# jesselasse/MARL-DMFB

Measured on AMD Instinct MI355X. Metric: env-steps/sec (whole node), 10x10 DMFB 4-droplet fov9, higher is better.
Workload: dtype int8 env state/obs + f64 rewards; fp32 Q-net; 1 GPU; DMFB 10x10, drop_num=4, fov=9, 4096 parallel envs per GPU (BASELINE configs[1]); parallelism=dp1: chips sharded per rank, one flat RCCL all-reduce per learn

## Files before the change

__graft_entry__.py:

```python
import os
import subprocess
import sys

ROOT = os.path.dirname(os.path.abspath(__file__))
if ROOT not in sys.path:
    sys.path.insert(0, ROOT)


def build():
    jobs = str(max(1, min(8, os.cpu_count() or 1)))
    env = dict(os.environ, PYTORCH_ROCM_ARCH='gfx950')
    subprocess.check_call(['make', '-C', os.path.join(ROOT, 'marl_dmfb_amd', 'csrc'), '-j', jobs, '-s'], env=env)
    subprocess.check_call(['make', '-C', os.path.join(ROOT, 'oracle'), '-s'], env=env)
    import marl_dmfb_amd
    from marl_dmfb_amd import _lib
    lib = _lib.dmfb_vec()
    for name in _lib.DMFB_VEC_SYMBOLS:
        getattr(lib, name)
    lib = _lib.meda_vec()
    for name in _lib.MEDA_VEC_SYMBOLS:
        getattr(lib, name)
    lib = _lib.crnn_ops()
    for name in ('crnn_conv9_forward', 'crnn_front9_forward', 'crnn_front19_forward', 'crnn_front_padded_cols', 'crnn_conv9_backward', 'crnn_conv19_backward', 'crnn_front9_forward_live', 'gru_seq_forward', 'gru_seq_backward', 'gru_seq_forward_packed', 'gru_seq_backward_packed'):
        getattr(lib, name)
    lib = _lib.crnn_fov()
    for name in _lib.SIGNATURES['crnn_fov']:
        getattr(lib, name)
    lib = _lib.crnn_wide()
    for name in _lib.SIGNATURES['crnn_wide']:
        getattr(lib, name)
    lib = _lib.rollout_ops()
    for name in ('rollout_select_actions', 'rollout_post_step', 'rollout_gru_head_select_stream', 'rollout_stream_step'):
        getattr(lib, name)
    lib = _lib.vdn_ops()
    for name in ('vdn_td_forward', 'vdn_td_backward', 'vdn_td_forward_packed', 'vdn_td_backward_packed', 'vdn_gather_units', 'vdn_clip_adam_step'):
        getattr(lib, name)
    for name in list(_lib.SIGNATURES['vdn_tail']) + list(_lib.SIGNATURES['vdn_lambda']) + list(_lib.SIGNATURES['vdn_double']):
        getattr(lib, name)
    lib = _lib.qmix_ops()
    for name in list(_lib.SIGNATURES['qmix_ops']) + list(_lib.SIGNATURES['qmix_packed']) + list(_lib.SIGNATURES['qmix_lambda']) + \
            list(_lib.SIGNATURES['qmix_double']):
        getattr(lib, name)
    lib = _lib.route_plan()
    for name in _lib.SIGNATURES['route_plan']:
        getattr(lib, name)
    lib = _lib.meda_plan()
# ... 82 lines not shown
```

marl_dmfb_amd/_lib.py:

```python
import ctypes as C
import os

_HERE = os.path.dirname(os.path.abspath(__file__))
LIB_DIR = os.path.join(_HERE, 'lib')
_CACHE = {}
_FILE = {'rollout_route': 'rollout_ops', 'vdn_tail': 'vdn_ops', 'vdn_lambda': 'vdn_ops', 'vdn_double': 'vdn_ops',
         'qmix_packed': 'qmix_ops', 'qmix_lambda': 'qmix_ops', 'qmix_double': 'qmix_ops'}


class HipLibraryMissing(RuntimeError):
    pass


def load(name):
    if name in _CACHE:
        return _CACHE[name]
    stem = _FILE.get(name, name)
    path = os.path.join(LIB_DIR, 'lib%s%s.so' % (stem, os.environ.get('MARL_DMFB_VARIANT_' + stem.upper(), '')))
    if not os.path.exists(path):
        raise HipLibraryMissing(
            '%s not found: build the HIP extension first (python -c "import __graft_entry__ as g; g.build()" '
            'or make -C marl_dmfb_amd/csrc). There is no CPU fallback.' % path)
    import torch
    lib = C.CDLL(path)
    _CACHE[name] = lib
    return lib


class DmfbVecConfig(C.Structure):
# ... 128 lines not shown
        'crnn_wide_last_hip_error': ([], i32),
    },
    'crnn_ops': {
        'crnn_conv9_forward': [vp, i64, i64, vp, vp, vp, vp, i32, vp, i64, vp],
        'crnn_front9_forward': [vp, i64, vp, i32, i64, vp, vp, vp, vp, vp, vp, i32, vp, i64, i32, vp],
        'crnn_front9_forward_live': [vp, i64, vp, i32, i64, vp, vp, vp, vp, vp, vp, i32, vp, i64, i32, vp, vp, i32, vp],
        'crnn_front19_forward': [vp, i64, vp, i32, i64, vp, vp, vp, vp, vp, vp, i32, vp, i64, i32, vp],
        'crnn_front_padded_cols': ([i32], i32),
        'crnn_conv9_backward_parts': ([i32], i32),
        'crnn_conv9_backward': [vp, i64, i64, vp, i64, vp, i64, vp, vp, vp, i32, vp, i32, vp, vp],
        'crnn_mlp_backward_parts': ([], i32),
        'crnn_mlp_backward': [vp, i64, i32, vp, i32, i64, vp, i64, vp, i64, i32, vp, vp, vp, vp],
        'crnn_conv19_backward_parts': ([i32], i32),
        'crnn_conv19_backward': [vp, i64, i64, vp, i64, vp, i64, vp, vp, vp, vp, i32, vp, i32, vp, vp],
        'crnn_last_hip_error': ([], i32),
        'gru_seq_forward': [vp, vp, vp, vp, vp, i32, i64, i32, vp, vp, vp],
        'gru_seq_backward': [vp, vp, vp, vp, vp, i32, i64, i32, vp, vp, vp, vp, vp],
        'gru_seq_forward_packed': [vp, vp, vp, vp, vp, i32, i64, i32, _i32p, vp, vp, vp],
        'gru_seq_forward_packed_pair': [vp] * 14 + [i32, i64, i32, _i32p, vp],
        'gru_seq_backward_packed': [vp, vp, vp, vp, vp, i32, i64, i32, _i32p, vp, vp, vp, vp, vp, vp],
        'gru_seq_row_blocks': ([i64], i64),
        'gru_last_hip_error': ([], i32),
    },
    'rollout_ops': {
        'rollout_select_actions': [vp, i32, i32, i32, vp, i32, u64, vp, vp, vp, vp, vp, i32, i32, vp],
        'rollout_gru_head_select': [vp, vp, vp, vp, vp, vp, vp, i32, i32, i32, i32, vp, i32, u64, vp, vp, vp, vp, vp, i32, i32, vp, vp],
        'rollout_gru_head_select_live': [vp, vp, vp, vp, vp, vp, vp, i32, i32, i32, i32, vp, i32, u64, vp, vp, vp, vp, vp, i32, i32, vp, vp,
                                         vp, vp],
        'rollout_compact_alive': [i32, vp, vp, vp, vp],
        'rollout_post_step': [i32, i32, i32, vp, vp, vp, vp, i32, vp, vp, vp, vp, vp, vp, vp, vp, vp, f32, f32, vp, vp, vp, i32, vp, vp,
                              vp],
        'rollout_gru_head_select_stream': [vp, vp, vp, vp, vp, vp, vp, i32, i32, i32, i32, vp, i32, u64, vp, vp, vp, vp, vp, i32, vp, vp,
                                           vp],
        'rollout_stream_step': [i32, i32, i32, i32, i32, i32, vp, vp, vp, vp, vp, vp, i32, vp, C.POINTER(RolloutStage),
                                C.POINTER(RolloutRing), i32, vp, vp, vp, f32, f32, vp, vp],
        'rollout_last_hip_error': ([], i32),
    },
    'rollout_route': {
        'rollout_route_select': [i32, i32, i32, i32, vp, vp, vp, i32, vp, vp, vp, vp, vp, vp],
        'rollout_last_hip_error': ([], i32),
    },
    'route_plan': {
        'route_plan_dmfb': [i32, i32, i32, i32, i32, vp, vp, vp, vp, vp, vp, vp, vp, vp, vp, vp],
        'route_follow_dmfb': [i32] * 6 + [vp] * 16,
        'route_plan_dmfb_opt': [i32] * 5 + [vp] * 10 + [i32, i32, vp],
        'route_follow_dmfb_opt': [i32] * 6 + [vp] * 15 + [i32, i32, vp],
# ... 193 lines not shown
    return _CACHE[key]


def dmfb_vec():
    return _library('dmfb_vec')


def meda_vec():
    return _library('meda_vec')


def crnn_ops():
    return _library('crnn_ops')


def crnn_fov():
    return _library('crnn_fov')


def crnn_wide():
    return _library('crnn_wide')


def rollout_ops():
    return _library('rollout_ops')


def rollout_route():
    return _library('rollout_route')


def route_plan():
    return _library('route_plan')


def meda_plan():
    return _library('meda_plan')


def meda_follow():
    return _library('meda_follow')


def meda_plan_wide():
    return _library('meda_plan_wide')

# ... 36 lines not shown
```

marl_dmfb_amd/csrc/gru_ops.hip:

```cpp
#include <hip/hip_runtime.h>

#include <cstdint>
#include <cstdio>
#include <cstdlib>

#include "../../include/crnn_ops.h"

#define HIP_ABI_TAG "crnn_ops"
#define HIP_ABI_ERR CRNN_ERR_HIP
#include "hip_abi.h"

namespace {

constexpr int kBlock = 512;
constexpr int H = 128;
constexpr int RW = 8;
constexpr int KQ = 32;

__device__ __forceinline__ float sigmoidf_(float x) { return 1.0f / (1.0f + __expf(-x)); }

struct SeqOff {
    int32_t packed;
    int32_t off[GRU_SEQ_MAX_STEPS + 1];
};

typedef float f32x2 __attribute__((ext_vector_type(2)));
typedef float f32x4 __attribute__((ext_vector_type(4)));

__global__ __launch_bounds__(kBlock) void k_gru_seq_fwd(const float *__restrict__ igates, const float *__restrict__ h0,
// ... 57 lines not shown
            const int rr = ra + s;
            if (rr < rvt) {
                const float hr = s_part[0][rr][0][u] + s_part[1][rr][0][u] + s_part[2][rr][0][u] + s_part[3][rr][0][u];
                const float hz = s_part[0][rr][1][u] + s_part[1][rr][1][u] + s_part[2][rr][1][u] + s_part[3][rr][1][u];
                const float hn = s_part[0][rr][2][u] + s_part[1][rr][2][u] + s_part[2][rr][2][u] + s_part[3][rr][2][u] + bhn;
                const float rg = sigmoidf_(ig[s][0] + hr + bir);
                const float zg = sigmoidf_(ig[s][1] + hz + biz);
                const float ng = tanhf(ig[s][2] + bin + rg * hn);
                const float hp = s_h[rr >> 1][u][rr & 1];
                const float hnew = (1.0f - zg) * ng + zg * hp;
                const size_t o = base + row0 + rr;
                hs[o * H + u] = hnew;
                if (gates) {
                    gates[o * 4 * H + u] = rg; gates[o * 4 * H + H + u] = zg; gates[o * 4 * H + 2 * H + u] = ng;
                    gates[o * 4 * H + 3 * H + u] = hn;
                }
                s_h[rr >> 1][u][rr & 1] = hnew;
            }
        }
        __syncthreads();
    }
}

__global__ __launch_bounds__(kBlock) void k_gru_seq_bwd(const float *__restrict__ grad_hs, const float *__restrict__ gates,
                                                        const float *__restrict__ hs, const float *__restrict__ h0,
                                                        const float *__restrict__ w_hh, int T, long R,
                                                        float *__restrict__ d_ig, float *__restrict__ d_hg,
                                                        float *__restrict__ d_h0, float *__restrict__ bias_part, const SeqOff so,
                                                        float *__restrict__ h_prev_out) {
    __shared__ __attribute__((aligned(16))) float s_dhg[RW / 2][3][H][2];
    __shared__ __attribute__((aligned(16))) float s_part[4][RW][H];
    const int tid = threadIdx.x, q = tid / H, u = tid - q * H;
    const long row0 = (long)blockIdx.x * RW;
    const int rv = (int)min((long)RW, R - row0);
    f32x4 wt[3][KQ / 4];
#pragma unroll
    for (int g = 0; g < 3; ++g)
#pragma unroll
        for (int k = 0; k < KQ / 4; ++k) {
            const float *col = w_hh + (size_t)(g * H + q * KQ + 4 * k) * H + u;
            wt[g][k] = (f32x4){col[0], col[H], col[2 * H], col[3 * H]};
        }
    const int ra = 2 * q;
    float gh[2] = {0.0f, 0.0f};
    float bs_r = 0.0f, bs_z = 0.0f, bs_n = 0.0f, bs_hn = 0.0f;
    int t_last = -1;
    for (int t = 0; t < T; ++t)
        if (row0 < (so.packed ? (long)(so.off[t + 1] - so.off[t]) : R)) t_last = t;
    struct In { float g, rg, zg, ng, hn, hp; };
    In cur[2], nx[2];
    auto fetch = [&](int t, In (&in)[2]) __attribute__((always_inline)) {
        const long rt = so.packed ? (long)(so.off[t + 1] - so.off[t]) : R;
        const int rvt = (int)min((long)rv, rt - row0);
        const size_t base = so.packed ? (size_t)so.off[t] : (size_t)t * R;
        const size_t base_prev = so.packed ? (size_t)so.off[t > 0 ? t - 1 : 0] : (size_t)(t > 0 ? t - 1 : 0) * R;
#pragma unroll
        for (int s = 0; s < 2; ++s) {
            const int rr = ra + s;
            const bool on = rr < rvt;
            const size_t o = base + row0 + (on ? rr : 0);
            in[s].g = on ? grad_hs[o * H + u] : 0.0f;
            in[s].rg = on ? gates[o * 4 * H + u] : 0.0f;
            in[s].zg = on ? gates[o * 4 * H + H + u] : 0.0f;
            in[s].ng = on ? gates[o * 4 * H + 2 * H + u] : 0.0f;
            in[s].hn = on ? gates[o * 4 * H + 3 * H + u] : 0.0f;
            in[s].hp = !on ? 0.0f : t > 0 ? hs[(base_prev + row0 + rr) * H + u] : h0 ? h0[(row0 + rr) * H + u] : 0.0f;
        }
    };
    if (t_last >= 0) fetch(t_last, cur);
    for (int t = t_last; t >= 0; --t) {
        const long rt = so.packed ? (long)(so.off[t + 1] - so.off[t]) : R;
        const int rvt = (int)min((long)rv, rt - row0);
        const size_t base = so.packed ? (size_t)so.off[t] : (size_t)t * R;
        float direct[2];
#pragma unroll
        for (int s = 0; s < 2; ++s) {
            const int rr = ra + s;
            float dpr = 0.0f, dpz = 0.0f, dpn = 0.0f, dhn = 0.0f;
            direct[s] = 0.0f;
            if (rr < rvt) {
                const size_t o = base + row0 + rr;
                const float g = cur[s].g + gh[s];
                const float rg = cur[s].rg, zg = cur[s].zg, ng = cur[s].ng, hn = cur[s].hn;
                const float hp = cur[s].hp;
                if (h_prev_out) h_prev_out[o * H + u] = hp;
                const float dn = g * (1.0f - zg), dz = g * (hp - ng);
                direct[s] = g * zg;
                dpn = dn * (1.0f - ng * ng);
                dhn = dpn * rg;
                dpr = dpn * hn * rg * (1.0f - rg);
                dpz = dz * zg * (1.0f - zg);
                d_ig[o * 3 * H + u] = dpr; d_ig[o * 3 * H + H + u] = dpz; d_ig[o * 3 * H + 2 * H + u] = dpn;
// ... 3 lines not shown
            s_dhg[rr >> 1][0][u][rr & 1] = dpr; s_dhg[rr >> 1][1][u][rr & 1] = dpz; s_dhg[rr >> 1][2][u][rr & 1] = dhn;
        }
        if (t > 0) fetch(t - 1, nx);
        __syncthreads();
#pragma unroll
        for (int rp = 0; rp < RW / 2; ++rp) {
            f32x2 acc = {0.0f, 0.0f};
#pragma unroll
            for (int g = 0; g < 3; ++g) {
                const f32x4 *pd = (const f32x4 *)(&s_dhg[rp][g][q * KQ][0]);
#pragma unroll
                for (int j = 0; j < KQ / 4; ++j) {
                    const f32x4 v0 = pd[2 * j], v1 = pd[2 * j + 1], wv = wt[g][j];
                    acc = __builtin_elementwise_fma((f32x2){wv.x, wv.x}, (f32x2){v0.x, v0.y}, acc);
                    acc = __builtin_elementwise_fma((f32x2){wv.y, wv.y}, (f32x2){v0.z, v0.w}, acc);
                    acc = __builtin_elementwise_fma((f32x2){wv.z, wv.z}, (f32x2){v1.x, v1.y}, acc);
                    acc = __builtin_elementwise_fma((f32x2){wv.w, wv.w}, (f32x2){v1.z, v1.w}, acc);
                }
            }
            s_part[q][2 * rp][u] = acc.x;
            s_part[q][2 * rp + 1][u] = acc.y;
        }
        __syncthreads();
#pragma unroll
        for (int s = 0; s < 2; ++s) {
            const int rr = ra + s;
            gh[s] = direct[s] + s_part[0][rr][u] + s_part[1][rr][u] + s_part[2][rr][u] + s_part[3][rr][u];
            cur[s] = nx[s];
        }
    }
    if (d_h0)
#pragma unroll
        for (int s = 0; s < 2; ++s)
            if (ra + s < rv) d_h0[(row0 + ra + s) * H + u] = gh[s];
    if (bias_part) {
        __syncthreads();
        s_part[q][0][u] = bs_r; s_part[q][1][u] = bs_z; s_part[q][2][u] = bs_n; s_part[q][3][u] = bs_hn;
        __syncthreads();
        if (q == 0) {
            float v[4];
#pragma unroll
            for (int k = 0; k < 4; ++k) v[k] = (s_part[0][k][u] + s_part[1][k][u]) + (s_part[2][k][u] + s_part[3][k][u]);
            float *bp = bias_part + (size_t)blockIdx.x * 6 * H;
            bp[u] = v[0]; bp[H + u] = v[1]; bp[2 * H + u] = v[2];
            bp[3 * H + u] = v[0]; bp[4 * H + u] = v[1]; bp[5 * H + u] = v[3];
        }
    }
}

constexpr int kMW = 16, kMHS = 132;
struct GruNetIO {
    const float *igates, *h0, *w_hh, *b_ih, *b_hh;
    float *hs, *gates;
};
__global__ __launch_bounds__(kBlock) void k_gru_seq_fwd_mfma(GruNetIO n0, GruNetIO n1, int blocks_per_net, int T, long R, const SeqOff so) {
    __shared__ __attribute__((aligned(16))) float s_h[2][kMW][kMHS];
    const bool second = (int)blockIdx.x >= blocks_per_net;
    const GruNetIO io = second ? n1 : n0;
    const long row0 = (long)((int)blockIdx.x - (second ? blocks_per_net : 0)) * kMW;
    const int tid = threadIdx.x, lane = tid & 63, wave = tid >> 6, j = lane & 15, kq = lane >> 4;
    const int u = 16 * wave + j;
    const int rv = (int)min((long)kMW, R - row0);
    f32x4 bw[3][8];
#pragma unroll
    for (int g = 0; g < 3; ++g)
#pragma unroll
        for (int jj = 0; jj < 8; ++jj) bw[g][jj] = *(const f32x4 *)(io.w_hh + (size_t)(g * H + u) * H + 16 * jj + 4 * kq);
    const float bir = io.b_ih[u] + io.b_hh[u], biz = io.b_ih[H + u] + io.b_hh[H + u], bin = io.b_ih[2 * H + u], bhn = io.b_hh[2 * H + u];
    for (int i = tid; i < kMW * H; i += kBlock) {
        const int rr = i / H, c = i - rr * H;
        s_h[0][rr][c] = (rr < rv && io.h0) ? io.h0[(row0 + rr) * H + c] : 0.0f;
        s_h[1][rr][c] = 0.0f;
    }
    __syncthreads();
    for (int t = 0; t < T; ++t) {
        const long rt = so.packed ? (long)(so.off[t + 1] - so.off[t]) : R;
        if (row0 >= rt) break;
        const int rvt = (int)min((long)rv, rt - row0);
        const size_t base = (so.packed ? (size_t)so.off[t] : (size_t)t * R) + (size_t)row0;
        const float (*cur)[kMHS] = s_h[t & 1];
        float (*nxt)[kMHS] = s_h[(t + 1) & 1];
        float ig[4][3];
#pragma unroll
        for (int q = 0; q < 4; ++q) {
            const int rr = 4 * kq + q;
#pragma unroll
            for (int g = 0; g < 3; ++g) ig[q][g] = rr < rvt ? io.igates[(base + rr) * 3 * H + g * H + u] : 0.0f;
        }
        f32x4 a4[8];
#pragma unroll
        for (int jj = 0; jj < 8; ++jj) a4[jj] = *(const f32x4 *)(&cur[j][16 * jj + 4 * kq]);
        f32x4 acc2[2][3];
#pragma unroll
        for (int hlf = 0; hlf < 2; ++hlf)
#pragma unroll
            for (int g = 0; g < 3; ++g) acc2[hlf][g] = f32x4{0.0f, 0.0f, 0.0f, 0.0f};
#pragma unroll
        for (int jj = 0; jj < 4; ++jj)
#pragma unroll
            for (int c = 0; c < 4; ++c)
#pragma unroll
                for (int hlf = 0; hlf < 2; ++hlf)
#pragma unroll
                    for (int g = 0; g < 3; ++g)
                        acc2[hlf][g] = __builtin_amdgcn_mfma_f32_16x16x4f32(a4[4 * hlf + jj][c], bw[g][4 * hlf + jj][c], acc2[hlf][g], 0, 0, 0);
        f32x4 acc[3];
#pragma unroll
        for (int g = 0; g < 3; ++g) acc[g] = acc2[0][g] + acc2[1][g];
#pragma unroll
        for (int q = 0; q < 4; ++q) {
            const int rr = 4 * kq + q;
            if (rr < rvt) {
                const float hn = acc[2][q] + bhn;
                const float rg = sigmoidf_(ig[q][0] + acc[0][q] + bir);
                const float zg = sigmoidf_(ig[q][1] + acc[1][q] + biz);
                const float ng = tanhf(ig[q][2] + bin + rg * hn);
                const float hp = cur[rr][u];
                const float hnew = (1.0f - zg) * ng + zg * hp;
                const size_t o = base + rr;
                io.hs[o * H + u] = hnew;
                if (io.gates) {
                    io.gates[o * 4 * H + u] = rg; io.gates[o * 4 * H + H + u] = zg; io.gates[o * 4 * H + 2 * H + u] = ng;
                    io.gates[o * 4 * H + 3 * H + u] = hn;
                }
                nxt[rr][u] = hnew;
            }
        }
        __syncthreads();
    }
}

}

extern "C" {

static int make_seq_off(const int32_t *step_rows, int T, int64_t R, SeqOff &so) {
    so.packed = step_rows ? 1 : 0;
    if (!step_rows) return CRNN_OK;
    if (T > GRU_SEQ_MAX_STEPS) return CRNN_ERR_UNSUPPORTED;
    long off = 0, prev = R;
    for (int t = 0; t < T; ++t) {
        if (step_rows[t] < 0 || step_rows[t] > prev) return CRNN_ERR_BAD_ARG;
        so.off[t] = (int32_t)off;
        off += step_rows[t];
        prev = step_rows[t];
        if (off > 0x7fffffffL) return CRNN_ERR_BAD_ARG;
    }
    so.off[T] = (int32_t)off;
    return CRNN_OK;
}

// ... 18 lines not shown
int gru_seq_forward_packed(const float *d_igates, const float *d_h0, const float *d_w_hh, const float *d_b_ih, const float *d_b_hh,
                           int T, int64_t R, int hidden, const int32_t *step_rows, float *d_hs, float *d_gates, void *stream) {
    if (!step_rows) return CRNN_ERR_BAD_ARG;
    return seq_forward(d_igates, d_h0, d_w_hh, d_b_ih, d_b_hh, T, R, hidden, step_rows, d_hs, d_gates, stream);
}

int gru_seq_forward_packed_pair(const float *d_igates_a, const float *d_h0_a, const float *d_w_hh_a, const float *d_b_ih_a,
                                const float *d_b_hh_a, float *d_hs_a, float *d_gates_a, const float *d_igates_b, const float *d_h0_b,
                                const float *d_w_hh_b, const float *d_b_ih_b, const float *d_b_hh_b, float *d_hs_b, float *d_gates_b,
                                int T, int64_t R, int hidden, const int32_t *step_rows, void *stream) {
    if (!d_igates_a || !d_w_hh_a || !d_b_ih_a || !d_b_hh_a || !d_hs_a || T < 0 || R < 0 || !step_rows) return CRNN_ERR_BAD_ARG;
    const bool two = d_igates_b != nullptr;
    if (two && (!d_w_hh_b || !d_b_ih_b || !d_b_hh_b || !d_hs_b)) return CRNN_ERR_BAD_ARG;
    if ((((size_t)d_w_hh_a | (size_t)d_w_hh_b) & 15) != 0) return CRNN_ERR_BAD_ARG;
    if (hidden != H) return CRNN_ERR_UNSUPPORTED;
    if (T == 0 || R == 0) return CRNN_OK;
    SeqOff so;
    const int rc = make_seq_off(step_rows, T, R, so);
    if (rc != CRNN_OK) return rc;
    const long per_net = (R + kMW - 1) / kMW;
    if (per_net * 2 > 0x7fffffffL) return CRNN_ERR_BAD_ARG;
    const GruNetIO a{d_igates_a, d_h0_a, d_w_hh_a, d_b_ih_a, d_b_hh_a, d_hs_a, d_gates_a};
    const GruNetIO b{d_igates_b, d_h0_b, d_w_hh_b, d_b_ih_b, d_b_hh_b, d_hs_b, d_gates_b};
    LAUNCH(k_gru_seq_fwd_mfma, dim3((unsigned)(per_net * (two ? 2 : 1))), dim3(kBlock), 0, (hipStream_t)stream, a, two ? b : a,
           (int)per_net, T, (long)R, so);
    return CRNN_OK;
}

static int seq_backward(const float *d_grad_hs, const float *d_gates, const float *d_hs, const float *d_h0, const float *d_w_hh,
                        int T, int64_t R, int hidden, const int32_t *step_rows, float *d_d_igates, float *d_d_hgates, float *d_d_h0,
                        float *d_bias_part, void *stream, float *d_h_prev = nullptr) {
    if (!d_grad_hs || !d_gates || !d_hs || !d_w_hh || !d_d_igates || !d_d_hgates || T < 0 || R < 0) return CRNN_ERR_BAD_ARG;
    if (hidden != H) return CRNN_ERR_UNSUPPORTED;
    if (T == 0 || R == 0) return CRNN_OK;
    SeqOff so;
    const int rc = make_seq_off(step_rows, T, R, so);
    if (rc != CRNN_OK) return rc;
    LAUNCH(k_gru_seq_bwd, dim3((unsigned)((R + RW - 1) / RW)), dim3(kBlock), 0, (hipStream_t)stream, d_grad_hs, d_gates, d_hs,
           d_h0, d_w_hh, T, (long)R, d_d_igates, d_d_hgates, d_d_h0, d_bias_part, so, d_h_prev);
    return CRNN_OK;
}

int gru_seq_backward(const float *d_grad_hs, const float *d_gates, const float *d_hs, const float *d_h0, const float *d_w_hh,
                     int T, int64_t R, int hidden, float *d_d_igates, float *d_d_hgates, float *d_d_h0, float *d_bias_part,
                     void *stream) {
    return seq_backward(d_grad_hs, d_gates, d_hs, d_h0, d_w_hh, T, R, hidden, nullptr, d_d_igates, d_d_hgates, d_d_h0, d_bias_part, stream);
}

int gru_seq_backward_packed(const float *d_grad_hs, const float *d_gates, const float *d_hs, const float *d_h0, const float *d_w_hh,
                            int T, int64_t R, int hidden, const int32_t *step_rows, float *d_d_igates, float *d_d_hgates,
                            float *d_d_h0, float *d_bias_part, float *d_h_prev, void *stream) {
    if (!step_rows) return CRNN_ERR_BAD_ARG;
    return seq_backward(d_grad_hs, d_gates, d_hs, d_h0, d_w_hh, T, R, hidden, step_rows, d_d_igates, d_d_hgates, d_d_h0, d_bias_part, stream,
                        d_h_prev);
}

int64_t gru_seq_row_blocks(int64_t R) { return (R + RW - 1) / RW; }

int gru_last_hip_error(void) { return g_last_hip; }

}
```

marl_dmfb_amd/network/base_net.py:

```python

import torch
import torch.nn as nn
import torch.nn.functional as f


_CONV_PLAN = {5: [(True, 1)], 7: [(True, 1), (False, 1)], 9: [(True, 1), (False, 1)], 11: [(True, 1), (False, 1)],
              13: [(True, 1), (False, 1)], 19: [(True, 2), (False, 1), (False, 1)]}


class _ConvGemm(torch.autograd.Function):

    @staticmethod
    def forward(ctx, cols, weight2d, bias):
        ctx.save_for_backward(cols, weight2d)
        return torch.addmm(bias, cols, weight2d.t())

    @staticmethod
    def backward(ctx, g):
        cols, w = ctx.saved_tensors
        g = g.contiguous()
        gcols = g @ w if ctx.needs_input_grad[0] else None
        M, K = cols.shape
        C = g.shape[1]
        S = 1
# ... 369 lines not shown
        Vp, G = igates.shape
        H, T, R, V = G // 3, len(step_rows), int(R) if h0 is None else h0.shape[0], int(sum(step_rows))
        igates, w_hh = igates.contiguous(), w_hh.contiguous()
        h0 = None if h0 is None else h0.contiguous()
        hs = torch.empty((Vp, H), dtype=torch.float32, device=igates.device)
        hs[V:].zero_()
        gates = torch.empty((Vp, 4 * H), dtype=torch.float32, device=igates.device) if save else None
        lib.gru_seq_forward_packed(igates.data_ptr(), None if h0 is None else h0.data_ptr(), w_hh.data_ptr(), b_ih.data_ptr(),
                                   b_hh.data_ptr(), T, R, H, _GRUSeqHipPacked._steps(step_rows), hs.data_ptr(),
                                   gates.data_ptr() if save else None,
                                   torch.cuda.current_stream(igates.device).cuda_stream)
        return hs, gates

    @staticmethod
    def forward(ctx, igates, h0, w_hh, b_ih, b_hh, step_rows, R=None):
        hs, gates = _GRUSeqHipPacked.run_forward(igates.detach(), None if h0 is None else h0.detach(), w_hh.detach(), b_ih.detach(),
                                                 b_hh.detach(), step_rows, True, R)
        ctx.save_for_backward(hs, gates, h0, w_hh)
        ctx.step_rows = list(step_rows)
        ctx.R = int(R) if h0 is None else h0.shape[0]
        return hs

    @staticmethod
    def backward(ctx, grad_out):
        hs, gates, h0, w_hh = ctx.saved_tensors
        lib = _GRUSeqHip._lib()
        step_rows = ctx.step_rows
        Vp, H = hs.shape
        T, R, V = len(step_rows), ctx.R, int(sum(step_rows))
        grad_out = grad_out.contiguous()
        h0c, w = None if h0 is None else h0.contiguous(), w_hh.contiguous()
        d_ig = torch.empty((Vp, 3 * H), dtype=torch.float32, device=hs.device)
        d_hg = torch.empty_like(d_ig)
        h_prev = torch.empty((Vp, H), dtype=torch.float32, device=hs.device)
        for t in (d_ig, d_hg, h_prev):
            t[V:].zero_()
        d_h0 = None if h0c is None else torch.zeros_like(h0c)
        bias_part = torch.empty((lib.gru_seq_row_blocks(R), 6 * H), dtype=torch.float32, device=hs.device)
        lib.gru_seq_backward_packed(grad_out.data_ptr(), gates.data_ptr(), hs.data_ptr(), None if h0c is None else h0c.data_ptr(),
                                    w.data_ptr(), T, R, H, _GRUSeqHipPacked._steps(step_rows), d_ig.data_ptr(),
                                    d_hg.data_ptr(), None if d_h0 is None else d_h0.data_ptr(), bias_part.data_ptr(), h_prev.data_ptr(),
                                    torch.cuda.current_stream(hs.device).cuda_stream)
        d_w_hh = _wgrad_splitk(d_hg, h_prev)
        d_b = bias_part.sum(0)
        return d_ig, d_h0, d_w_hh, d_b[:3 * H], d_b[3 * H:], None, None


class _GRUSeqPairPacked(torch.autograd.Function):

    @staticmethod
    def forward(ctx, ig_a, w_hh_a, b_ih_a, b_hh_a, ig_b, w_hh_b, b_ih_b, b_hh_b, step_rows, R):
        lib = _GRUSeqHip._lib()
        Vp, G = ig_a.shape
        Hd, T, V = G // 3, len(step_rows), int(sum(step_rows))
        save = any(ctx.needs_input_grad[:4])
        ta = [t.detach().contiguous() for t in (ig_a, w_hh_a, b_ih_a, b_hh_a)]
        tb = [t.detach().contiguous() for t in (ig_b, w_hh_b, b_ih_b, b_hh_b)]
        hs_a = torch.empty((Vp, Hd), dtype=torch.float32, device=ig_a.device)
        hs_b = torch.empty((Vp, Hd), dtype=torch.float32, device=ig_a.device)
        hs_a[V:].zero_()
        hs_b[V:].zero_()
        gates = torch.empty((Vp, 4 * Hd), dtype=torch.float32, device=ig_a.device) if save else None
        lib.gru_seq_forward_packed_pair(ta[0].data_ptr(), None, ta[1].data_ptr(), ta[2].data_ptr(), ta[3].data_ptr(),
                                        hs_a.data_ptr(), gates.data_ptr() if save else None,
                                        tb[0].data_ptr(), None, tb[1].data_ptr(), tb[2].data_ptr(), tb[3].data_ptr(),
                                        hs_b.data_ptr(), None, T, R, Hd, _GRUSeqHipPacked._steps(step_rows),
                                        torch.cuda.current_stream(ig_a.device).cuda_stream)
        if save:
            ctx.save_for_backward(hs_a, gates, None, ta[1])
            ctx.step_rows = list(step_rows)
            ctx.R = int(R)
        ctx.mark_non_differentiable(hs_b)
        ctx.set_materialize_grads(False)
        return hs_a, hs_b

    @staticmethod
    def backward(ctx, grad_a, _grad_b):
        if grad_a is None:
            return (None,) * 10
        d_ig, _d_h0, d_w_hh, d_b_ih, d_b_hh, _, _ = _GRUSeqHipPacked.backward(ctx, grad_a)
        return d_ig, d_w_hh, d_b_ih, d_b_hh, None, None, None, None, None, None


def gru_sequence(igates, h0, w_hh, b_ih, b_hh, impl='hip'):
    if impl == 'hip' and h0.shape[-1] == 128 and igates.dtype == torch.float32:
        if torch.is_grad_enabled() and any(t.requires_grad for t in (igates, h0, w_hh, b_ih, b_hh)):
            return _GRUSeqHip.apply(igates, h0, w_hh, b_ih, b_hh)
        return _GRUSeqHip.run_forward(igates, h0, w_hh, b_ih, b_hh, False)[0]
    return _GRUSeq.apply(igates, h0, w_hh, b_ih, b_hh)


def conv_str(fov, id=3, od=32):
    stack, shared = [], None
    for from_image, stride in _CONV_PLAN[fov]:
        if from_image:
            stack.append(nn.Conv2d(id, od, kernel_size=3, stride=stride))
        else:
            if shared is None:
                shared = nn.Conv2d(od, od, kernel_size=3, stride=stride)
            stack.append(shared)
    return stack


class CRNN(nn.Module):
    def __init__(self, args):
        super().__init__()
# ... 63 lines not shown
        q = self.fc1(torch.stack(hs, dim=0).view(T * R, -1)).view(T, R, -1)
        return q, h

    def recurrent_seq_packed(self, x, step_rows, R, return_hidden=False):
        w_ih = self.weight_ih_padded() if x.shape[-1] == self.padded_cols() != self.rnn.weight_ih.shape[1] else self.rnn.weight_ih
        igates = _LinearSplitK.apply(x, w_ih, None)
        args = (igates, None, self.rnn.weight_hh, self.rnn.bias_ih, self.rnn.bias_hh)
        if torch.is_grad_enabled() and any(t.requires_grad for t in args if t is not None):
            hs = _GRUSeqHipPacked.apply(*args, step_rows, R)
        else:
            hs = _GRUSeqHipPacked.run_forward(*args, step_rows, False, R)[0]
        q = _LinearSplitK.apply(hs, self.fc1.weight, self.fc1.bias)
        return (q, hs.detach()) if return_hidden else q

    @staticmethod
    def recurrent_seq_packed_pair(net_a, x_a, net_b, x_b, step_rows, R, return_hidden=False):
        def w_ih(net, x, grad):
            if x.shape[-1] == net.padded_cols() != net.rnn.weight_ih.shape[1]:
                return net.weight_ih_padded() if grad else net.refresh_padded()
            return net.rnn.weight_ih
        ig_a = _LinearSplitK.apply(x_a, w_ih(net_a, x_a, True), None)
        with torch.no_grad():
            ig_b = torch.matmul(x_b, w_ih(net_b, x_b, False).t())
        hs_a, hs_b = _GRUSeqPairPacked.apply(ig_a, net_a.rnn.weight_hh, net_a.rnn.bias_ih, net_a.rnn.bias_hh,
                                             ig_b, net_b.rnn.weight_hh.detach(), net_b.rnn.bias_ih.detach(), net_b.rnn.bias_hh.detach(),
                                             step_rows, R)
        q_a = _LinearSplitK.apply(hs_a, net_a.fc1.weight, net_a.fc1.bias)
        with torch.no_grad():
            q_b = torch.addmm(net_b.fc1.bias, hs_b, net_b.fc1.weight.t())
        return (q_a, q_b, hs_a.detach()) if return_hidden else (q_a, q_b)

    def forward(self, inputs, hidden_state):
        return self.recurrent(self.features(inputs), hidden_state)

    def _pixel_features_hip(self, obs_i8):
        from .. import _lib
        lib = _lib.checked('crnn_ops')
        obs_i8 = obs_i8.contiguous()
        geo = self._hip_front()
        if geo in (5, 7):
            return _fov_front_forward(self, obs_i8, None, self.out, vec=False)
        if geo in (11, 13):
            return _wide_front_forward(self, obs_i8, None, self.out, vec=False)
        R = obs_i8.shape[0]
        out = torch.empty((R, self.out), dtype=torch.float32, device=obs_i8.device)
        c1, c2 = self.convs[0], self.convs[1]
# ... 162 lines not shown
```

Measured before the change: 7.919 million env-steps/s.

## Fuse Q-head linear layer into packed GRU sequence forward and backward kernels

Adds templated GRU kernels that compute the fc1 Q-head inside the recurrent loop. In the forward pass the head for step t-1 overlaps with the MFMA work of step t. In the backward pass dQ is read directly and projected back through fc1 with wave readlanes, so the separate hs gradient matmul is skipped. The target network no longer writes its hidden states to memory. This removes extra launches and hs round trips for the head GEMMs, at the cost of more shared memory, more registers, and a cap of 16 actions.

```diff
diff --git a/__graft_entry__.py b/__graft_entry__.py
--- a/__graft_entry__.py
+++ b/__graft_entry__.py
@@ -22,6 +22,9 @@
         getattr(lib, name)
     lib = _lib.crnn_ops()
     for name in ('crnn_conv9_forward', 'crnn_front9_forward', 'crnn_front19_forward', 'crnn_front_padded_cols', 'crnn_conv9_backward', 'crnn_conv19_backward', 'crnn_front9_forward_live', 'gru_seq_forward', 'gru_seq_backward', 'gru_seq_forward_packed', 'gru_seq_backward_packed'):
+        getattr(lib, name)
+    lib = _lib.gru_head()
+    for name in _lib.SIGNATURES['gru_head']:
         getattr(lib, name)
     lib = _lib.crnn_fov()
     for name in _lib.SIGNATURES['crnn_fov']:
diff --git a/include/gru_head.h b/include/gru_head.h
--- /dev/null
+++ b/include/gru_head.h
@@ -0,0 +1,23 @@
+#ifndef GRU_HEAD_H
+#define GRU_HEAD_H
+
+#include <stdint.h>
+
+#ifdef __cplusplus
+extern "C" {
+#endif
+
+int gru_head_forward_packed_pair(const float *d_igates_a, const float *d_h0_a, const float *d_w_hh_a, const float *d_b_ih_a,
+                                 const float *d_b_hh_a, float *d_hs_a, float *d_gates_a, const float *d_w_fc_a, const float *d_b_fc_a,
+                                 float *d_q_a, const float *d_igates_b, const float *d_h0_b, const float *d_w_hh_b,
+                                 const float *d_b_ih_b, const float *d_b_hh_b, float *d_hs_b, float *d_gates_b, const float *d_w_fc_b,
+                                 const float *d_b_fc_b, float *d_q_b, int n_actions, int T, int64_t R, int hidden,
+                                 const int32_t *step_rows, void *stream);
+int gru_head_backward_packed(const float *d_dq, const float *d_w_fc, int n_actions, const float *d_gates, const float *d_hs,
+                             const float *d_h0, const float *d_w_hh, int T, int64_t R, int hidden, const int32_t *step_rows,
+                             float *d_d_igates, float *d_d_hgates, float *d_d_h0, float *d_bias_part, float *d_h_prev, void *stream);
+
+#ifdef __cplusplus
+}
+#endif
+#endif
diff --git a/marl_dmfb_amd/_lib.py b/marl_dmfb_amd/_lib.py
--- a/marl_dmfb_amd/_lib.py
+++ b/marl_dmfb_amd/_lib.py
@@ -4,7 +4,7 @@
 _HERE = os.path.dirname(os.path.abspath(__file__))
 LIB_DIR = os.path.join(_HERE, 'lib')
 _CACHE = {}
-_FILE = {'rollout_route': 'rollout_ops', 'vdn_tail': 'vdn_ops', 'vdn_lambda': 'vdn_ops', 'vdn_double': 'vdn_ops',
+_FILE = {'gru_head': 'crnn_ops', 'rollout_route': 'rollout_ops', 'vdn_tail': 'vdn_ops', 'vdn_lambda': 'vdn_ops', 'vdn_double': 'vdn_ops',
          'qmix_packed': 'qmix_ops', 'qmix_lambda': 'qmix_ops', 'qmix_double': 'qmix_ops'}
 
 
@@ -179,6 +179,10 @@
         'gru_seq_row_blocks': ([i64], i64),
         'gru_last_hip_error': ([], i32),
     },
+    'gru_head': {
+        'gru_head_forward_packed_pair': [vp] * 20 + [i32, i32, i64, i32, _i32p, vp],
+        'gru_head_backward_packed': [vp, vp, i32, vp, vp, vp, vp, i32, i64, i32, _i32p, vp, vp, vp, vp, vp, vp],
+    },
     'rollout_ops': {
         'rollout_select_actions': [vp, i32, i32, i32, vp, i32, u64, vp, vp, vp, vp, vp, i32, i32, vp],
         'rollout_gru_head_select': [vp, vp, vp, vp, vp, vp, vp, i32, i32, i32, i32, vp, i32, u64, vp, vp, vp, vp, vp, i32, i32, vp, vp],
@@ -418,6 +422,10 @@
     return _library('crnn_wide')
 
 
+def gru_head():
+    return _library('gru_head')
+
+
 def rollout_ops():
     return _library('rollout_ops')
 
diff --git a/marl_dmfb_amd/csrc/gru_ops.hip b/marl_dmfb_amd/csrc/gru_ops.hip
--- a/marl_dmfb_amd/csrc/gru_ops.hip
+++ b/marl_dmfb_amd/csrc/gru_ops.hip
@@ -3,8 +3,10 @@
 #include <cstdint>
 #include <cstdio>
 #include <cstdlib>
+#include <type_traits>
 
 #include "../../include/crnn_ops.h"
+#include "../../include/gru_head.h"
 
 #define HIP_ABI_TAG "crnn_ops"
 #define HIP_ABI_ERR CRNN_ERR_HIP
@@ -108,12 +110,14 @@
     }
 }
 
+constexpr int kMaxA = 16;
+template <bool HEAD>
 __global__ __launch_bounds__(kBlock) void k_gru_seq_bwd(const float *__restrict__ grad_hs, const float *__restrict__ gates,
                                                         const float *__restrict__ hs, const float *__restrict__ h0,
                                                         const float *__restrict__ w_hh, int T, long R,
                                                         float *__restrict__ d_ig, float *__restrict__ d_hg,
                                                         float *__restrict__ d_h0, float *__restrict__ bias_part, const SeqOff so,
-                                                        float *__restrict__ h_prev_out) {
+                                                        float *__restrict__ h_prev_out, const float *__restrict__ w_fc, int A) {
     __shared__ __attribute__((aligned(16))) float s_dhg[RW / 2][3][H][2];
     __shared__ __attribute__((aligned(16))) float s_part[4][RW][H];
     const int tid = threadIdx.x, q = tid / H, u = tid - q * H;
@@ -127,6 +131,15 @@
             const float *col = w_hh + (size_t)(g * H + q * KQ + 4 * k) * H + u;
             wt[g][k] = (f32x4){col[0], col[H], col[2 * H], col[3 * H]};
         }
+    __shared__ float s_wf[HEAD ? kMaxA : 1][H];
+    if constexpr (HEAD) {
+        float v[kMaxA * H / kBlock];
+#pragma unroll
+        for (int k = 0; k < kMaxA * H / kBlock; ++k) v[k] = tid + k * kBlock < A * H ? w_fc[tid + k * kBlock] : 0.0f;
+#pragma unroll
+        for (int k = 0; k < kMaxA * H / kBlock; ++k) s_wf[(tid + k * kBlock) / H][(tid + k * kBlock) % H] = v[k];
+        __syncthreads();
+    }
     const int ra = 2 * q;
     float gh[2] = {0.0f, 0.0f};
     float bs_r = 0.0f, bs_z = 0.0f, bs_n = 0.0f, bs_hn = 0.0f;
@@ -135,6 +148,23 @@
         if (row0 < (so.packed ? (long)(so.off[t + 1] - so.off[t]) : R)) t_last = t;
     struct In { float g, rg, zg, ng, hn, hp; };
     In cur[2], nx[2];
+    const int dq_lane = tid & 63;
+    auto head_chain = [&](In (&in)[2], auto n) __attribute__((always_inline)) {
+        float w[decltype(n)::value], g0 = 0.0f, g1 = 0.0f;
+#pragma unroll
+        for (int a = 0; a < decltype(n)::value; ++a) w[a] = s_wf[a][u];
+#pragma unroll
+        for (int a = 0; a < decltype(n)::value; ++a) {
+            g0 = __builtin_fmaf(__int_as_float(__builtin_amdgcn_readlane(__float_as_int(in[0].g), a)), w[a], g0);
+            g1 = __builtin_fmaf(__int_as_float(__builtin_amdgcn_readlane(__float_as_int(in[1].g), a)), w[a], g1);
+        }
+        in[0].g = g0;
+        in[1].g = g1;
+    };
+    auto head_grad = [&](In (&in)[2]) __attribute__((always_inline)) {
+        if (A <= 8) head_chain(in, std::integral_constant<int, 8>{});
+        else head_chain(in, std::integral_constant<int, kMaxA>{});
+    };
     auto fetch = [&](int t, In (&in)[2]) __attribute__((always_inline)) {
         const long rt = so.packed ? (long)(so.off[t + 1] - so.off[t]) : R;
         const int rvt = (int)min((long)rv, rt - row0);
@@ -145,7 +175,8 @@
             const int rr = ra + s;
             const bool on = rr < rvt;
             const size_t o = base + row0 + (on ? rr : 0);
-            in[s].g = on ? grad_hs[o * H + u] : 0.0f;
+            if constexpr (HEAD) in[s].g = on && dq_lane < A ? grad_hs[o * A + dq_lane] : 0.0f;
+            else in[s].g = on ? grad_hs[o * H + u] : 0.0f;
             in[s].rg = on ? gates[o * 4 * H + u] : 0.0f;
             in[s].zg = on ? gates[o * 4 * H + H + u] : 0.0f;
             in[s].ng = on ? gates[o * 4 * H + 2 * H + u] : 0.0f;
@@ -154,6 +185,7 @@
         }
     };
     if (t_last >= 0) fetch(t_last, cur);
+    if constexpr (HEAD) head_grad(cur);
     for (int t = t_last; t >= 0; --t) {
         const long rt = so.packed ? (long)(so.off[t + 1] - so.off[t]) : R;
         const int rvt = (int)min((long)rv, rt - row0);
@@ -203,6 +235,9 @@
             s_part[q][2 * rp + 1][u] = acc.y;
         }
         __syncthreads();
+        if constexpr (HEAD) {
+            if (t > 0) head_grad(nx);
+        }
 #pragma unroll
         for (int s = 0; s < 2; ++s) {
             const int rr = ra + s;
@@ -234,10 +269,19 @@
     const float *igates, *h0, *w_hh, *b_ih, *b_hh;
     float *hs, *gates;
 };
-__global__ __launch_bounds__(kBlock) void k_gru_seq_fwd_mfma(GruNetIO n0, GruNetIO n1, int blocks_per_net, int T, long R, const SeqOff so) {
+struct GruHeadIO {
+    const float *w, *b;
+    float *q;
+};
+template <bool HEAD>
+__global__ __launch_bounds__(kBlock) void k_gru_seq_fwd_mfma(GruNetIO n0, GruNetIO n1, int blocks_per_net, int T, long R, const SeqOff so,
+                                                             GruHeadIO hd0, GruHeadIO hd1, int A) {
     __shared__ __attribute__((aligned(16))) float s_h[2][kMW][kMHS];
+    __shared__ __attribute__((aligned(16))) float s_w[HEAD ? kMaxA : 1][kMHS];
+    __shared__ float s_b[kMaxA];
     const bool second = (int)blockIdx.x >= blocks_per_net;
     const GruNetIO io = second ? n1 : n0;
+    const GruHeadIO hd = second ? hd1 : hd0;
     const long row0 = (long)((int)blockIdx.x - (second ? blocks_per_net : 0)) * kMW;
     const int tid = threadIdx.x, lane = tid & 63, wave = tid >> 6, j = lane & 15, kq = lane >> 4;
     const int u = 16 * wave + j;
@@ -253,8 +297,43 @@
         s_h[0][rr][c] = (rr < rv && io.h0) ? io.h0[(row0 + rr) * H + c] : 0.0f;
         s_h[1][rr][c] = 0.0f;
     }
+    if constexpr (HEAD) {
+        float v[kMaxA * H / kBlock];
+#pragma unroll
+        for (int k = 0; k < kMaxA * H / kBlock; ++k) v[k] = tid + k * kBlock < A * H ? hd.w[tid + k * kBlock] : 0.0f;
+#pragma unroll
+        for (int k = 0; k < kMaxA * H / kBlock; ++k) s_w[(tid + k * kBlock) / H][(tid + k * kBlock) % H] = v[k];
+        if (tid < A) s_b[tid] = hd.b[tid];
+    }
     __syncthreads();
-    for (int t = 0; t < T; ++t) {
+    auto head = [&](const float (*hb)[kMHS], size_t base_p, int rv_p) __attribute__((always_inline)) {
+        const int rr = tid & (kMW - 1), a = tid >> 4;
+        if (tid < kMW * A && rr < rv_p) {
+            const f32x4 *ph = (const f32x4 *)(&hb[rr][0]), *pw = (const f32x4 *)(&s_w[a][0]);
+            float acc = s_b[a];
+            f32x4 hv[2][4], wv[2][4];
+#pragma unroll
+            for (int e = 0; e < 4; ++e) { hv[0][e] = ph[e]; wv[0][e] = pw[e]; }
+#pragma unroll
+            for (int k = 0; k < H / 16; ++k) {
+                if (k + 1 < H / 16) {
+#pragma unroll
+                    for (int e = 0; e < 4; ++e) { hv[(k + 1) & 1][e] = ph[4 * (k + 1) + e]; wv[(k + 1) & 1][e] = pw[4 * (k + 1) + e]; }
+                }
+#pragma unroll
+                for (int e = 0; e < 4; ++e) {
+                    acc = __builtin_fmaf(hv[k & 1][e].x, wv[k & 1][e].x, acc);
+                    acc = __builtin_fmaf(hv[k & 1][e].y, wv[k & 1][e].y, acc);
+                    acc = __builtin_fmaf(hv[k & 1][e].z, wv[k & 1][e].z, acc);
+                    acc = __builtin_fmaf(hv[k & 1][e].w, wv[k & 1][e].w, acc);
+                }
+            }
+            hd.q[(base_p + rr) * A + a] = acc;
+        }
+    };
+    int t = 0, rv_prev = 0;
+    size_t base_prev = 0;
+    for (; t < T; ++t) {
         const long rt = so.packed ? (long)(so.off[t + 1] - so.off[t]) : R;
         if (row0 >= rt) break;
         const int rvt = (int)min((long)rv, rt - row0);
@@ -285,6 +364,11 @@
 #pragma unroll
                     for (int g = 0; g < 3; ++g)
                         acc2[hlf][g] = __builtin_amdgcn_mfma_f32_16x16x4f32(a4[4 * hlf + jj][c], bw[g][4 * hlf + jj][c], acc2[hlf][g], 0, 0, 0);
+        if constexpr (HEAD) {
+            if (rv_prev > 0) head(cur, base_prev, rv_prev);
+            rv_prev = rvt;
+            base_prev = base;
+        }
         f32x4 acc[3];
 #pragma unroll
         for (int g = 0; g < 3; ++g) acc[g] = acc2[0][g] + acc2[1][g];
@@ -299,7 +383,7 @@
                 const float hp = cur[rr][u];
                 const float hnew = (1.0f - zg) * ng + zg * hp;
                 const size_t o = base + rr;
-                io.hs[o * H + u] = hnew;
+                if (!HEAD || io.hs) io.hs[o * H + u] = hnew;
                 if (io.gates) {
                     io.gates[o * 4 * H + u] = rg; io.gates[o * 4 * H + H + u] = zg; io.gates[o * 4 * H + 2 * H + u] = ng;
                     io.gates[o * 4 * H + 3 * H + u] = hn;
@@ -308,6 +392,9 @@
             }
         }
         __syncthreads();
+    }
+    if constexpr (HEAD) {
+        if (rv_prev > 0) head(s_h[t & 1], base_prev, rv_prev);
     }
 }
 
@@ -372,22 +459,56 @@
     if (per_net * 2 > 0x7fffffffL) return CRNN_ERR_BAD_ARG;
     const GruNetIO a{d_igates_a, d_h0_a, d_w_hh_a, d_b_ih_a, d_b_hh_a, d_hs_a, d_gates_a};
     const GruNetIO b{d_igates_b, d_h0_b, d_w_hh_b, d_b_ih_b, d_b_hh_b, d_hs_b, d_gates_b};
-    LAUNCH(k_gru_seq_fwd_mfma, dim3((unsigned)(per_net * (two ? 2 : 1))), dim3(kBlock), 0, (hipStream_t)stream, a, two ? b : a,
-           (int)per_net, T, (long)R, so);
+    LAUNCH(k_gru_seq_fwd_mfma<false>, dim3((unsigned)(per_net * (two ? 2 : 1))), dim3(kBlock), 0, (hipStream_t)stream, a, two ? b : a,
+           (int)per_net, T, (long)R, so, GruHeadIO{}, GruHeadIO{}, 0);
     return CRNN_OK;
 }
 
-static int seq_backward(const float *d_grad_hs, const float *d_gates, const float *d_hs, const float *d_h0, const float *d_w_hh,
-                        int T, int64_t R, int hidden, const int32_t *step_rows, float *d_d_igates, float *d_d_hgates, float *d_d_h0,
-                        float *d_bias_part, void *stream, float *d_h_prev = nullptr) {
-    if (!d_grad_hs || !d_gates || !d_hs || !d_w_hh || !d_d_igates || !d_d_hgates || T < 0 || R < 0) return CRNN_ERR_BAD_ARG;
+int gru_head_forward_packed_pair(const float *d_igates_a, const float *d_h0_a, const float *d_w_hh_a, const float *d_b_ih_a,
+                                     const float *d_b_hh_a, float *d_hs_a, float *d_gates_a, const float *d_w_fc_a, const float *d_b_fc_a,
+                                     float *d_q_a, const float *d_igates_b, const float *d_h0_b, const float *d_w_hh_b,
+                                     const float *d_b_ih_b, const float *d_b_hh_b, float *d_hs_b, float *d_gates_b, const float *d_w_fc_b,
+                                     const float *d_b_fc_b, float *d_q_b, int n_actions, int T, int64_t R, int hidden,
+                                     const int32_t *step_rows, void *stream) {
+    if (!d_igates_a || !d_w_hh_a || !d_b_ih_a || !d_b_hh_a || !d_hs_a || !d_w_fc_a || !d_b_fc_a || !d_q_a || T < 0 || R < 0 || !step_rows)
+        return CRNN_ERR_BAD_ARG;
+    if (n_actions < 1 || n_actions > kMaxA) return CRNN_ERR_BAD_ARG;
+    const bool two = d_igates_b != nullptr;
+    if (two && (!d_w_hh_b || !d_b_ih_b || !d_b_hh_b || !d_w_fc_b || !d_b_fc_b || !d_q_b)) return CRNN_ERR_BAD_ARG;
+    if ((((size_t)d_w_hh_a | (size_t)d_w_hh_b) & 15) != 0) return CRNN_ERR_BAD_ARG;
     if (hidden != H) return CRNN_ERR_UNSUPPORTED;
     if (T == 0 || R == 0) return CRNN_OK;
     SeqOff so;
     const int rc = make_seq_off(step_rows, T, R, so);
     if (rc != CRNN_OK) return rc;
-    LAUNCH(k_gru_seq_bwd, dim3((unsigned)((R + RW - 1) / RW)), dim3(kBlock), 0, (hipStream_t)stream, d_grad_hs, d_gates, d_hs,
-           d_h0, d_w_hh, T, (long)R, d_d_igates, d_d_hgates, d_d_h0, d_bias_part, so, d_h_prev);
+    const long per_net = (R + kMW - 1) / kMW;
+    if (per_net * 2 > 0x7fffffffL) return CRNN_ERR_BAD_ARG;
+    const GruNetIO a{d_igates_a, d_h0_a, d_w_hh_a, d_b_ih_a, d_b_hh_a, d_hs_a, d_gates_a};
+    const GruNetIO b{d_igates_b, d_h0_b, d_w_hh_b, d_b_ih_b, d_b_hh_b, d_hs_b, d_gates_b};
+    const GruHeadIO ha{d_w_fc_a, d_b_fc_a, d_q_a}, hb{d_w_fc_b, d_b_fc_b, d_q_b};
+    LAUNCH(k_gru_seq_fwd_mfma<true>, dim3((unsigned)(per_net * (two ? 2 : 1))), dim3(kBlock), 0, (hipStream_t)stream, a, two ? b : a,
+           (int)per_net, T, (long)R, so, ha, two ? hb : ha, n_actions);
+    return CRNN_OK;
+}
+
+static int seq_backward(const float *d_grad_hs, const float *d_gates, const float *d_hs, const float *d_h0, const float *d_w_hh,
+                        int T, int64_t R, int hidden, const int32_t *step_rows, float *d_d_igates, float *d_d_hgates, float *d_d_h0,
+                        float *d_bias_part, void *stream, float *d_h_prev = nullptr, const float *d_w_fc = nullptr, int n_actions = 0) {
+    if (!d_grad_hs || !d_gates || !d_hs || !d_w_hh || !d_d_igates || !d_d_hgates || T < 0 || R < 0) return CRNN_ERR_BAD_ARG;
+    if (d_w_fc && (n_actions < 1 || n_actions > kMaxA)) return CRNN_ERR_BAD_ARG;
+    if (hidden != H) return CRNN_ERR_UNSUPPORTED;
+    if (T == 0 || R == 0) return CRNN_OK;
+    SeqOff so;
+    const int rc = make_seq_off(step_rows, T, R, so);
+    if (rc != CRNN_OK) return rc;
+    const dim3 grid((unsigned)((R + RW - 1) / RW));
+    if (d_w_fc) {
+        LAUNCH(k_gru_seq_bwd<true>, grid, dim3(kBlock), 0, (hipStream_t)stream, d_grad_hs, d_gates, d_hs, d_h0, d_w_hh, T, (long)R,
+               d_d_igates, d_d_hgates, d_d_h0, d_bias_part, so, d_h_prev, d_w_fc, n_actions);
+    } else {
+        LAUNCH(k_gru_seq_bwd<false>, grid, dim3(kBlock), 0, (hipStream_t)stream, d_grad_hs, d_gates, d_hs, d_h0, d_w_hh, T, (long)R,
+               d_d_igates, d_d_hgates, d_d_h0, d_bias_part, so, d_h_prev, (const float *)nullptr, 1);
+    }
     return CRNN_OK;
 }
 
@@ -405,6 +526,14 @@
                         d_h_prev);
 }
 
+int gru_head_backward_packed(const float *d_dq, const float *d_w_fc, int n_actions, const float *d_gates, const float *d_hs,
+                                 const float *d_h0, const float *d_w_hh, int T, int64_t R, int hidden, const int32_t *step_rows,
+                                 float *d_d_igates, float *d_d_hgates, float *d_d_h0, float *d_bias_part, float *d_h_prev, void *stream) {
+    if (!step_rows || !d_w_fc) return CRNN_ERR_BAD_ARG;
+    return seq_backward(d_dq, d_gates, d_hs, d_h0, d_w_hh, T, R, hidden, step_rows, d_d_igates, d_d_hgates, d_d_h0, d_bias_part, stream,
+                        d_h_prev, d_w_fc, n_actions);
+}
+
 int64_t gru_seq_row_blocks(int64_t R) { return (R + RW - 1) / RW; }
 
 int gru_last_hip_error(void) { return g_last_hip; }
diff --git a/marl_dmfb_amd/network/base_net.py b/marl_dmfb_amd/network/base_net.py
--- a/marl_dmfb_amd/network/base_net.py
+++ b/marl_dmfb_amd/network/base_net.py
@@ -1,3 +1,4 @@
+import os
 
 import torch
 import torch.nn as nn
@@ -415,8 +416,8 @@
         return hs
 
     @staticmethod
-    def backward(ctx, grad_out):
-        hs, gates, h0, w_hh = ctx.saved_tensors
+    def backward(ctx, grad_out, head_w=None):
+        hs, gates, h0, w_hh = ctx.saved_tensors[:4]
         lib = _GRUSeqHip._lib()
         step_rows = ctx.step_rows
         Vp, H = hs.shape
@@ -430,10 +431,15 @@
             t[V:].zero_()
         d_h0 = None if h0c is None else torch.zeros_like(h0c)
         bias_part = torch.empty((lib.gru_seq_row_blocks(R), 6 * H), dtype=torch.float32, device=hs.device)
-        lib.gru_seq_backward_packed(grad_out.data_ptr(), gates.data_ptr(), hs.data_ptr(), None if h0c is None else h0c.data_ptr(),
-                                    w.data_ptr(), T, R, H, _GRUSeqHipPacked._steps(step_rows), d_ig.data_ptr(),
-                                    d_hg.data_ptr(), None if d_h0 is None else d_h0.data_ptr(), bias_part.data_ptr(), h_prev.data_ptr(),
-                                    torch.cuda.current_stream(hs.device).cuda_stream)
+        tail = (None if h0c is None else h0c.data_ptr(), w.data_ptr(), T, R, H, _GRUSeqHipPacked._steps(step_rows), d_ig.data_ptr(),
+                d_hg.data_ptr(), None if d_h0 is None else d_h0.data_ptr(), bias_part.data_ptr(), h_prev.data_ptr(),
+                torch.cuda.current_stream(hs.device).cuda_stream)
+        if head_w is None:
+            lib.gru_seq_backward_packed(grad_out.data_ptr(), gates.data_ptr(), hs.data_ptr(), *tail)
+        else:
+            from .. import _lib
+            _lib.checked('gru_head').gru_head_backward_packed(grad_out.data_ptr(), head_w.data_ptr(), head_w.shape[0], gates.data_ptr(),
+                                                              hs.data_ptr(), *tail)
         d_w_hh = _wgrad_splitk(d_hg, h_prev)
         d_b = bias_part.sum(0)
         return d_ig, d_h0, d_w_hh, d_b[:3 * H], d_b[3 * H:], None, None
@@ -475,6 +481,48 @@
         return d_ig, d_w_hh, d_b_ih, d_b_hh, None, None, None, None, None, None
 
 
+class _GRUHeadPairPacked(torch.autograd.Function):
+
+    @staticmethod
+    def forward(ctx, ig_a, w_hh_a, b_ih_a, b_hh_a, w_fc_a, b_fc_a, ig_b, w_hh_b, b_ih_b, b_hh_b, w_fc_b, b_fc_b, step_rows, R):
+        from .. import _lib
+        lib = _lib.checked('gru_head')
+        Vp, G = ig_a.shape
+        Hd, T, V, A = G // 3, len(step_rows), int(sum(step_rows)), w_fc_a.shape[0]
+        save = any(ctx.needs_input_grad[:6])
+        ta = [t.detach().contiguous() for t in (ig_a, w_hh_a, b_ih_a, b_hh_a, w_fc_a, b_fc_a)]
+        tb = [t.detach().contiguous() for t in (ig_b, w_hh_b, b_ih_b, b_hh_b, w_fc_b, b_fc_b)]
+        dev = ig_a.device
+        hs_a = torch.empty((Vp, Hd), dtype=torch.float32, device=dev)
+        q_a = torch.empty((Vp, A), dtype=torch.float32, device=dev)
+        q_b = torch.empty((Vp, A), dtype=torch.float32, device=dev)
+        if Vp > V:
+            for t in (hs_a, q_a, q_b):
+                t[V:].zero_()
+        gates = torch.empty((Vp, 4 * Hd), dtype=torch.float32, device=dev) if save else None
+        lib.gru_head_forward_packed_pair(ta[0].data_ptr(), None, ta[1].data_ptr(), ta[2].data_ptr(), ta[3].data_ptr(), hs_a.data_ptr(),
+                                         gates.data_ptr() if save else None, ta[4].data_ptr(), ta[5].data_ptr(), q_a.data_ptr(),
+                                         tb[0].data_ptr(), None, tb[1].data_ptr(), tb[2].data_ptr(), tb[3].data_ptr(), None, None,
+                                         tb[4].data_ptr(), tb[5].data_ptr(), q_b.data_ptr(), A, T, R, Hd,
+                                         _GRUSeqHipPacked._steps(step_rows), torch.cuda.current_stream(dev).cuda_stream)
+        if save:
+            ctx.save_for_backward(hs_a, gates, None, ta[1], ta[4])
+            ctx.step_rows = list(step_rows)
+            ctx.R = int(R)
+        ctx.mark_non_differentiable(q_b, hs_a)
+        ctx.set_materialize_grads(False)
+        return q_a, q_b, hs_a
+
+    @staticmethod
+    def backward(ctx, dq, _dq_b, _dhs):
+        if dq is None:
+            return (None,) * 14
+        dq = dq.contiguous()
+        hs_a, w_fc = ctx.saved_tensors[0], ctx.saved_tensors[4]
+        d_ig, _d_h0, d_w_hh, d_b_ih, d_b_hh, _, _ = _GRUSeqHipPacked.backward(ctx, dq, head_w=w_fc)
+        return (d_ig, d_w_hh, d_b_ih, d_b_hh, _wgrad_splitk(dq, hs_a), _colsum(dq)) + (None,) * 8
+
+
 def gru_sequence(igates, h0, w_hh, b_ih, b_hh, impl='hip'):
     if impl == 'hip' and h0.shape[-1] == 128 and igates.dtype == torch.float32:
         if torch.is_grad_enabled() and any(t.requires_grad for t in (igates, h0, w_hh, b_ih, b_hh)):
@@ -584,6 +632,12 @@
         ig_a = _LinearSplitK.apply(x_a, w_ih(net_a, x_a, True), None)
         with torch.no_grad():
             ig_b = torch.matmul(x_b, w_ih(net_b, x_b, False).t())
+        if os.environ.get('MARL_DMFB_GRU_HEAD', '1') != '0' and net_a.fc1.weight.shape[0] <= 16:
+            q_a, q_b, hs_a = _GRUHeadPairPacked.apply(ig_a, net_a.rnn.weight_hh, net_a.rnn.bias_ih, net_a.rnn.bias_hh, net_a.fc1.weight,
+                                                      net_a.fc1.bias, ig_b, net_b.rnn.weight_hh.detach(), net_b.rnn.bias_ih.detach(),
+                                                      net_b.rnn.bias_hh.detach(), net_b.fc1.weight.detach(), net_b.fc1.bias.detach(),
+                                                      step_rows, R)
+            return (q_a, q_b, hs_a) if return_hidden else (q_a, q_b)
         hs_a, hs_b = _GRUSeqPairPacked.apply(ig_a, net_a.rnn.weight_hh, net_a.rnn.bias_ih, net_a.rnn.bias_hh,
                                              ig_b, net_b.rnn.weight_hh.detach(), net_b.rnn.bias_ih.detach(), net_b.rnn.bias_hh.detach(),
                                              step_rows, R)
```

After: 7.903 million env-steps/s. Within noise of the previous version (-0.2%).
